# yoyololicon/pytorch-NMF

Measured on AMD Instinct MI355X. Metric: MU GFLOP/s (algorithmic 8*N*C*R per iteration), dense NMF 4096x65536 rank-128 beta=1; MU iterations/s alongside, higher is better.
Workload: dtype f16; 1 GPU; NMF 4096x65536 rank=128 beta=1 (BASELINE configs[1]); preset=cfg1, rows=4096, cols_per_gpu=65536, rank=128, precision=f16, parallelism=single GPU, nsplit_h=16, nsplit_w=1, block_rows_h=256, block_rows_w=256, launch=eager launches

## Files before the change

include/nmfmu.h:

```cpp
#ifndef NMFMU_H_
#define NMFMU_H_

#include <stddef.h>
#include <stdint.h>

#ifdef __cplusplus
extern "C" {
#endif

#define NMFMU_ABI_VERSION 9

#define NMFMU_OK 0
#define NMFMU_ERR_UNSUPPORTED (-2)
#define NMFMU_ERR_ARG (-3)
#define NMFMU_ERR_ALLOC (-4)

#define NMFMU_PREC_BF16 0
#define NMFMU_PREC_BF16X3 1
#define NMFMU_PREC_F16 2
#define NMFMU_PREC_F16X 3
#define NMFMU_PREC_F16R 4

#define NMFMU_BETA_KL 0
#define NMFMU_BETA_EUC 1
#define NMFMU_BETA_IS 2
#define NMFMU_BETA_GEN 3

#define NMFMU_STAGE_REG 0
#define NMFMU_STAGE_DMA 1
#define NMFMU_STAGE_DMA_NOP2 3
#define NMFMU_STAGE_DMA_SPLIT 2

typedef struct nmfmu_factor {
  float* f;
  void* p1_hi;
  void* p1_lo;
  void* p2_hi;
  void* p2_lo;
  float* colsum;
  float* colsum_part;
  int32_t rows;
  int32_t rows_pad;
} nmfmu_factor;

typedef struct nmfmu_step {
// ... 15 lines not shown
  void* stamps;
} nmfmu_step;

int nmfmu_abi_version(void);
int nmfmu_abi_check(int compiled_against);
int nmfmu_pad_rows(int rows);
int nmfmu_pad_rank(int rank);
int nmfmu_beta_kind(float beta);
int nmfmu_supported(int r_pad, int precision);
int nmfmu_block_rows(int r_pad, int precision, float beta);
int nmfmu_choose_nsplit(int owner_rows_pad, int panel_rows_pad, int block_rows, int num_cu);
#define NMFMU_KERNEL_FUSED 0
#define NMFMU_KERNEL_PP 1
#define NMFMU_KERNEL_SP 2
int nmfmu_kernel_family(int r_pad, int precision, float beta);
int nmfmu_choose_nsplit_for(int owner_rows_pad, int panel_rows_pad, int r_pad, int precision, float beta, int block_rows, int num_cu);
int nmfmu_step_block_rows(int owner_rows_pad, int panel_rows_pad, int r_pad, int precision, float beta, int num_cu);
size_t nmfmu_xp_bytes(int owner_rows_pad, int panel_rows_pad, int precision);
size_t nmfmu_image_bytes(int rows_pad, int r_pad);
size_t nmfmu_slab_bytes(int owner_rows_pad, int r_pad, int nsplit);
size_t nmfmu_colsum_part_bytes(int rows_pad, int r_pad);

int nmfmu_pack_x(const float* v, int64_t ld, int rows, int cols, int transpose, int precision, int block_rows, void* xp,
                 int owner_rows_pad, int panel_rows_pad, uint32_t* flags, void* stream);

int nmfmu_pack_factor(const nmfmu_factor* fac, int rank, int r_pad, int precision, void* stream);

int nmfmu_pack_factor_scaled(const nmfmu_factor* fac, int rank, int r_pad, int precision, const float* scale,
                             void* stream);

// ... 244 lines not shown
```

pytorch-nmf_amd/csrc/nmfmu_capi.hip:

```cpp
#include <hip/hip_runtime.h>
#include <stdint.h>

#include <algorithm>
#include <cstdlib>
#include <new>
#include <vector>

#include "../../include/nmfmu.h"
#include "nmfmu_aux.h"
#include "nmfmu_fused.h"
#include "nmfmu_pp.h"
#include "nmfmu_sp.h"
#include "nmfmu_sp2.h"

#ifndef NMFMU_SP
#define NMFMU_SP 1
#endif
#ifndef NMFMU_SP2
#define NMFMU_SP2 1
#endif
#ifndef NMFMU_FUSE_APPLY_TWO_ACC
#define NMFMU_FUSE_APPLY_TWO_ACC 1
#endif

// ... 9 lines not shown

#ifdef NMFMU_DEBUG_HOOKS
static int env_int(const char* name, int dflt) {
  const char* v = std::getenv(name);
  return v && *v ? std::atoi(v) : dflt;
}
static void* g_pp_debug = nullptr;
#endif
#ifndef NMFMU_PP_F16R
#define NMFMU_PP_F16R 1
#endif
static bool pp_eligible(int r_pad, int precision, float beta) {
  return nmfmu_beta_kind(beta) == NMFMU_BETA_KL && r_pad <= 128 &&
         (precision == NMFMU_PREC_F16 || precision == NMFMU_PREC_BF16 || (NMFMU_PP_F16R && precision == NMFMU_PREC_F16R));
}
static bool sp_eligible(int r_pad, int precision, float beta) {
  return NMFMU_SP && nmfmu_beta_kind(beta) == NMFMU_BETA_KL && r_pad == 256 && precision == NMFMU_PREC_F16;
}
static bool sp2_eligible(int r_pad, int precision, float beta) {
  const int k = nmfmu_beta_kind(beta);
  return NMFMU_SP2 && (k == NMFMU_BETA_IS || k == NMFMU_BETA_GEN) && r_pad == 128 && precision == NMFMU_PREC_F16;
}
static int kernel_beta_kind(float beta) {
  if (beta == 0.5f) return kSqrt;
  if (beta == 1.5f) return kSqrt3;
  return nmfmu_beta_kind(beta);
}

struct GramRef {
  const float* gram;
  const void* hi;
  const void* lo;
  const float* scale;
};

int fused_dispatch(const nmfmu_step* st, int mode, float* loss_part, int M, int K, hipStream_t s,
                   const float* fuse_kl_den = nullptr, bool fuse_apply = false, const GramRef* gm = nullptr) {
  if (!st || !st->owner.p1_hi || !st->panel.p1_hi) return NMFMU_ERR_ARG;
  if (!st->xp && (mode == kModeMU || mode == kModeXB)) return NMFMU_ERR_ARG;
  if (st->owner.rows_pad % kRowPad || st->panel.rows_pad % kRowPad) return NMFMU_ERR_ARG;
  if (st->block_rows != 128 && st->block_rows != 256) return NMFMU_ERR_ARG;
  if (st->stage != NMFMU_STAGE_DMA && st->stage != NMFMU_STAGE_DMA_SPLIT && st->stage != NMFMU_STAGE_DMA_NOP2)
    return NMFMU_ERR_UNSUPPORTED;
  if (st->stage == NMFMU_STAGE_DMA_SPLIT && mode == kModeMU && !(st->precision == NMFMU_PREC_BF16X3)) {
    if (nmfmu_beta_kind(st->beta) != NMFMU_BETA_KL || st->block_rows != 128) return NMFMU_ERR_UNSUPPORTED;
    mode = kModeMU2;
  }
  if (st->r_pad != pad_rank(st->rank) || st->nsplit < 1) return NMFMU_ERR_ARG;
  const bool x3 = st->precision == NMFMU_PREC_BF16X3;
  if (x3 && (!st->owner.p1_lo || !st->panel.p1_lo)) return NMFMU_ERR_ARG;
  const int kind = nmfmu_beta_kind(st->beta);
  if (st->precision == NMFMU_PREC_F16R && kind == NMFMU_BETA_EUC) return NMFMU_ERR_UNSUPPORTED;
  FusedArgs a{};
  a.xp = st->xp;
  a.p1_hi = static_cast<const uint16_t*>(st->panel.p1_hi);
  a.p1_lo = static_cast<const uint16_t*>(st->panel.p1_lo);
  a.p2_hi = static_cast<const uint16_t*>(st->panel.p2_hi);
// ... 39 lines not shown
  } else if (mode == kModeMU || mode == kModeDen) {
    if (!a.slab_num || !a.p2_hi || (x3 && !a.p2_lo)) return NMFMU_ERR_ARG;
    if (mode == kModeMU && kind != kKL && !a.slab_den) return NMFMU_ERR_ARG;
    if (mode == kModeDen && (kind != kGen || st->block_rows != 128)) return NMFMU_ERR_UNSUPPORTED;
  } else if (!loss_part) {
    return NMFMU_ERR_ARG;
  }
  const int grid = (st->owner.rows_pad / st->block_rows) * st->nsplit;
  if (st->block_rows == 256) {
    if (!st->xp || mode == kModeDen || !pp_eligible(st->r_pad, st->precision, st->beta)) return NMFMU_ERR_UNSUPPORTED;
    a.tiles_per_split = (a.tiles_per_split + 1) & ~1;
    a.debug = mode == kModeMU ? st->stamps : nullptr;
#ifdef NMFMU_DEBUG_HOOKS
    if (mode == kModeMU && g_pp_debug) a.debug = g_pp_debug;
#endif
    return launch_pp(st->r_pad, is_f16(st->precision) ? kOpF16 : kOpBf16, mode, a, grid, s, st->precision == NMFMU_PREC_F16R,
                      mode == kModeMU && loss_part != nullptr);
  }
  if (mode == kModeMU && sp_eligible(st->r_pad, st->precision, st->beta)) {
    a.tiles_per_split = (a.tiles_per_split + 3) & ~3;
    a.debug = st->stamps;
#ifdef NMFMU_DEBUG_HOOKS
    if (g_pp_debug) a.debug = g_pp_debug;
#endif
    if (st->stage == NMFMU_STAGE_DMA_NOP2) a.o2_hi = nullptr;
    return launch_sp(st->r_pad, kOpF16, a, grid, s);
  }
  if (mode == kModeMU && sp2_eligible(st->r_pad, st->precision, st->beta)) {
    a.tiles_per_split = (a.tiles_per_split + 3) & ~3;
    return launch_sp2(st->r_pad, kernel_beta_kind(st->beta), a, grid, s);
  }
  const int kk = kernel_beta_kind(st->beta);
// ... 52 lines not shown
  static const int forced = env_int("NMFMU_FORCE_NSPLIT", 0);
  if (forced > 0) return std::min(forced, std::max(1, ktiles));
#endif
  const int target = (block_rows == 128 ? 2 : 1) * std::max(num_cu, 1);
  int ns = (target + mblocks - 1) / mblocks;
  if (ns > 8) ns = (ns + 7) / 8 * 8;
  ns = std::min(ns, std::max(1, ktiles / 4));
  return std::max(ns, 1);
}

int nmfmu_kernel_family(int r_pad, int precision, float beta) {
  if (pp_eligible(r_pad, precision, beta)) return NMFMU_KERNEL_PP;
  if (sp_eligible(r_pad, precision, beta) || sp2_eligible(r_pad, precision, beta)) return NMFMU_KERNEL_SP;
  return NMFMU_KERNEL_FUSED;
}

int nmfmu_choose_nsplit_for(int owner_rows_pad, int panel_rows_pad, int r_pad, int precision, float beta, int block_rows, int num_cu) {
  if (owner_rows_pad <= 0 || panel_rows_pad <= 0 || (block_rows != 128 && block_rows != 256)) return NMFMU_ERR_ARG;
  if (block_rows == 128 && (sp_eligible(r_pad, precision, beta) || sp2_eligible(r_pad, precision, beta))) {
    const int mblocks = owner_rows_pad / 128, ktiles = panel_rows_pad / kBK;
    int ns = (std::max(num_cu, 1) + mblocks - 1) / mblocks;
    ns = std::min(ns, std::max(1, ktiles / 8));
    return std::max(ns, 1);
  }
  return nmfmu_choose_nsplit(owner_rows_pad, panel_rows_pad, block_rows, num_cu);
}

int nmfmu_step_block_rows(int owner_rows_pad, int panel_rows_pad, int r_pad, int precision, float beta, int num_cu) {
  if (pp_eligible(r_pad, precision, beta)) return 256;
  if (owner_rows_pad <= 0 || panel_rows_pad <= 0) return NMFMU_ERR_ARG;
// ... 117 lines not shown
  a.nslab = num ? nslab : st->nsplit;
  a.kl_den = kl ? kl_den : nullptr;
  if (!a.num || a.nslab < 1) return NMFMU_ERR_ARG;
  a.den_nslab = den_nslab;
  a.skip_colsum = skip_colsum;
  if (kl ? !a.kl_den : !a.den) return NMFMU_ERR_ARG;
  a.p1_hi = st->owner.p1_hi, a.p1_lo = st->owner.p1_lo, a.p2_hi = st->owner.p2_hi, a.p2_lo = st->owner.p2_lo;
  a.colsum_part = st->owner.colsum_part, a.colsum = st->owner.colsum;
  a.rows = st->owner.rows, a.rank = st->rank, a.rows_pad = st->owner.rows_pad;
  a.l1 = st->l1, a.l2 = st->l2, a.gamma = st->gamma;
  a.trainer = trainer, a.ortho = ortho, a.grad = grad;
  a.f16 = is_f16(st->precision);
  a.status = st->status;
  if (!a.p1_hi || !a.p2_hi || !a.colsum || !a.colsum_part) return NMFMU_ERR_ARG;
  if (st->stage == NMFMU_STAGE_DMA_NOP2 && sp_eligible(st->r_pad, st->precision, st->beta)) a.p2_hi = a.p2_lo = nullptr;
  return launch_apply(st->r_pad, a, st->precision == NMFMU_PREC_BF16X3, false, S(stream));
}

int nmfmu_mu_apply(const nmfmu_step* st, const float* num, const float* den, int nslab, const float* kl_den,
                   void* stream) {
  return apply_common(st, num, den, nslab, kl_den, 0, 0.f, nullptr, stream);
}

int nmfmu_trainer_apply(const nmfmu_step* st, const float* num, const float* den, int nslab, const float* kl_den,
                        float ortho, float* grad, void* stream) {
  if (!(ortho >= 0.f)) return NMFMU_ERR_ARG;
  return apply_common(st, num, den, nslab, kl_den, 1, ortho, grad, stream);
}

int nmfmu_xb_supported(int r_pad, int precision, float beta) {
// ... 233 lines not shown
```

pytorch-nmf_amd/csrc/nmfmu_inst_pp.hip:

```cpp
#include "nmfmu_pp.h"

namespace nmfmu {

bool pp_available(int r_pad, int opt, int mode) {
  return (r_pad == 32 || r_pad == 64 || r_pad == 128) && (opt == kOpBf16 || opt == kOpF16) &&
         (mode == kModeMU || mode == kModeLoss);
}

template <int R_PAD>
static int launch_pp_r(int opt, int mode, const FusedArgs& a, int grid, hipStream_t s, bool xr, bool lacc) {
  if (lacc) {
    if (opt != kOpF16 || mode != kModeMU || !a.loss_part) return -2;
    return xr ? launch_pp_one<R_PAD, kOpF16, kModeMU, true, true>(a, grid, s) : launch_pp_one<R_PAD, kOpF16, kModeMU, false, true>(a, grid, s);
  }
  if (xr) {
    if (opt == kOpF16 && mode == kModeMU) return launch_pp_one<R_PAD, kOpF16, kModeMU, true>(a, grid, s);
    if (opt == kOpF16 && mode == kModeLoss) return launch_pp_one<R_PAD, kOpF16, kModeLoss, true>(a, grid, s);
    return -2;
  }
  if (opt == kOpBf16 && mode == kModeMU) return launch_pp_one<R_PAD, kOpBf16, kModeMU>(a, grid, s);
  if (opt == kOpF16 && mode == kModeMU) return launch_pp_one<R_PAD, kOpF16, kModeMU>(a, grid, s);
  if (opt == kOpBf16 && mode == kModeLoss) return launch_pp_one<R_PAD, kOpBf16, kModeLoss>(a, grid, s);
  if (opt == kOpF16 && mode == kModeLoss) return launch_pp_one<R_PAD, kOpF16, kModeLoss>(a, grid, s);
  return -2;
}

int launch_pp(int r_pad, int opt, int mode, const FusedArgs& a, int grid, hipStream_t s, bool xr, bool lacc) {
  switch (r_pad) {
    case 32: return launch_pp_r<32>(opt, mode, a, grid, s, xr, lacc);
    case 64: return launch_pp_r<64>(opt, mode, a, grid, s, xr, lacc);
    case 128: return launch_pp_r<128>(opt, mode, a, grid, s, xr, lacc);
  }
  return -2;
}

}
```

pytorch-nmf_amd/csrc/nmfmu_pp.h:

```cpp
#pragma once
#include "nmfmu_fused.h"

#ifndef NMFMU_PP_DUP
#define NMFMU_PP_DUP 0
#endif
#ifndef NMFMU_PP_XM
#define NMFMU_PP_XM -1
#endif

namespace nmfmu {

template <int R_PAD, int OPT, int MODE, bool XR_ = false, bool LACC_ = false>
struct PPCfg {
  static constexpr int BM = 256, WAVES = 8, THREADS = 512;
  static constexpr int KS = R_PAD / 16;
  static constexpr int RT = R_PAD / 32;
  static constexpr int ROWB = 2 * R_PAD;
  static constexpr int IMG = kBK * ROWB;
  static constexpr bool LOSS = MODE == kModeLoss;
  static constexpr int LEAD = 2;
  static constexpr int NSLOT = 3;
  static constexpr bool XR = XR_;
  static constexpr int NX = XR ? 6 : 4;
  static constexpr int XTILE = BM * kBK * (XR ? 3 : 2);
  static_assert(!XR || OPT == kOpF16, "the 3-byte target comes with fp16 operands");
  static constexpr bool LACC = LACC_;
  static_assert(!LACC || (OPT == kOpF16 && MODE == kModeMU), "riding loss: fp16 operands, MU half-step");
  static constexpr bool XM = (NMFMU_PP_DUP & (4 | 32)) ? false : (NMFMU_PP_XM < 0 ? XR : NMFMU_PP_XM != 0);
  static constexpr int P1_BASE = 0, P2_BASE = NSLOT * IMG;
  static constexpr int LDS_MAIN = 2 * NSLOT * IMG;
  static constexpr int LDS_EPI = LOSS ? 64 : WAVES * 32 * R_PAD * 4;
  static constexpr int LDS_BYTES = LDS_MAIN > LDS_EPI ? LDS_MAIN : LDS_EPI;
  static constexpr int NPIECE = IMG / 1024;
  static constexpr int ND = (NPIECE + 3) / 4;
  static constexpr int NSTEP1 = 2 * KS, NSTEP2 = LOSS ? 0 : 4 * RT;
  static constexpr int PF = 4;
  static constexpr bool SCALED = OPT == kOpBf16;
  static_assert(NSTEP1 >= PF, "ring deeper than G1");
};

template <int R_PAD, int OPT, int MODE, bool XR = false, bool LACC = false>
__global__ void __launch_bounds__(512, 2) pp_kernel(const FusedArgs a) {
  using C = PPCfg<R_PAD, OPT, MODE, XR, LACC>;
  constexpr int NX = C::NX;
  constexpr int KS = C::KS, RT = C::RT, ROWB = C::ROWB, IMG = C::IMG, PF = C::PF;
  constexpr int NSTEP1 = C::NSTEP1, NSTEP2 = C::NSTEP2;
  extern __shared__ __attribute__((aligned(16))) char smem[];

  const int tid = threadIdx.x;
  const int lane = tid & 63;
  const int wave = __builtin_amdgcn_readfirstlane(tid >> 6);
  const int half = wave >> 2;
  const int j = lane & 31;
  const int hl = lane >> 5;
  const int mb = blockIdx.x / a.nsplit;
  const int ks = blockIdx.x - mb * a.nsplit;
  const int t0 = ks * a.tiles_per_split;
  const int t1 = min(t0 + a.tiles_per_split, a.ktiles);
// ... 93 lines not shown
#pragma unroll
      for (int i = 0; i < C::ND; ++i) {
        const unsigned pc = (4u * i) % (unsigned)C::NPIECE;
        if constexpr (C::NPIECE >= 4)
          dma1k(src_tile + pc * 1024u, pvoff, lds_base + lds_off + pc * 1024u + (unsigned)(wave & 3) * 1024u);
        else
          dma1k(src_tile, ((unsigned)(wave & 3) % (unsigned)C::NPIECE) * 1024u + lane16,
                lds_base + lds_off + ((unsigned)(wave & 3) % (unsigned)C::NPIECE) * 1024u);
      }
    };
    unsigned p1_issue_off = (unsigned)(C::LEAD % C::NSLOT) * IMG;
    unsigned p2_issue_off = (unsigned)((C::LEAD - 1) % C::NSLOT) * IMG;
    auto next_off = [&](unsigned off) { return off == (unsigned)(C::NSLOT - 1) * IMG ? 0u : off + IMG; };
    auto issue_panel = [&](int t) {
      dma_img(p1src + (size_t)clampt(t + C::LEAD) * IMG, C::P1_BASE + p1_issue_off);
      if constexpr (!C::LOSS) dma_img(p2src + (size_t)clampt(t + C::LEAD - 1) * IMG, C::P2_BASE + p2_issue_off);
    };
#ifdef NMFMU_PP_X_DEFAULT_POLICY
#define NMFMU_PP_XPOL ""
#else
#define NMFMU_PP_XPOL " nt"
#endif
    u32x4 xA[NX], xB[NX];
#if NMFMU_PP_DUP & (4 | 32)
    u32x4 xdupA[4], xdupB[4];
#if NMFMU_PP_DUP & 32
    const long long xmirror = (long long)((int)(gridDim.x / a.nsplit) - 1 - 2 * mb) * (long long)a.ktiles * (long long)C::XTILE;
#else
    const long long xmirror = 0;
#endif
#endif
// ... 70 lines not shown
    uint32_t gn[2][8];
    f32x16 S[2];
    u32x4 ring[PF];
#ifdef NMFMU_PP_ABLATE_STALE_OPERANDS
    u32x4 abl_sink = {0u, 0u, 0u, 0u};
#endif

    constexpr int BACK = (C::NSLOT - 1) * IMG;
    int sa[2] = {a_base[0] + C::P1_BASE, a_base[1] + C::P1_BASE};
    int sb[2][2];
#pragma unroll
    for (int tt = 0; tt < 2; ++tt)
#pragma unroll
      for (int m2 = 0; m2 < 2; ++m2) sb[tt][m2] = b_base[tt][m2] + C::P2_BASE + BACK;
    int rd1 = 0, rd2 = BACK;
    auto advance_slots = [&]() {
      const int d1 = rd1 == BACK ? -BACK : IMG;
      const int d2 = rd2 == BACK ? -BACK : IMG;
      rd1 += d1, rd2 += d2;
      sa[0] += d1, sa[1] += d1;
      if constexpr (!C::LOSS) {
#pragma unroll
        for (int tt = 0; tt < 2; ++tt)
#pragma unroll
          for (int m2 = 0; m2 < 2; ++m2) sb[tt][m2] += d2;
      }
    };
    auto rd = [&](u32x4& dst, int addr, auto offc) {
#if NMFMU_PP_DUP & 1
      asm volatile("ds_read_b128 %0, %1 offset:%2\n\tds_read_b128 %0, %1 offset:%2" : "=v"(dst) : "v"(addr), "n"(decltype(offc)::value));
#else
      asm volatile("ds_read_b128 %0, %1 offset:%2" : "=v"(dst) : "v"(addr), "n"(decltype(offc)::value));
#endif
    };
    auto opnd = [&](u32x4& dst, auto ec, auto g1c) {
// ... 74 lines not shown
          mma(acc[rt], nh, op);
        }
        if constexpr (e + PF < NS) opnd(ring[e % PF], std::integral_constant<int, e + PF>{}, g1c);
        if constexpr (decltype(fillc)::value) {
          static_for<NX>([&](auto ic) {
            if constexpr ((decltype(ic)::value * NS) / NX == e) fill(ic);
          });
        }
      });
      if constexpr (g1 && N2 == 0) asm volatile("s_nop 15\n\ts_nop 7" ::: "memory");
    };
    auto elementwise_segment = [&](int t, auto nextc, u32x4(&x)[NX], auto tailc) {
      constexpr bool next_has_g1 = decltype(nextc)::value;
      constexpr bool tail = decltype(tailc)::value;
      advance_slots();
      if constexpr (next_has_g1) prefetch(std::true_type{});
      else if constexpr (!C::LOSS) prefetch(std::false_type{});
      if constexpr (!tail) {
        if (!half) issue_panel(t);
      } else if constexpr (next_has_g1 && !C::LOSS) {
        if (!half) dma_img(p2src + (size_t)(t + 1) * IMG, C::P2_BASE + p2_issue_off);
      }
#pragma unroll
      for (int tt = 0; tt < 2; ++tt) {
        if constexpr (C::LOSS) {
#pragma unroll
          for (int d = 0; d < 8; ++d) {
            const uint32_t w = x[2 * tt + (d >> 2)][d & 3];
            float x0, x1;
            if constexpr (C::XR) {
              const uint32_t uw = x[4 + tt][d >> 1], j0 = 2 * (d & 1);
              x0 = __builtin_bit_cast(float, __builtin_amdgcn_perm(w, uw, 0x0504000cu | (j0 << 8)));
              x1 = __builtin_bit_cast(float, __builtin_amdgcn_perm(w, uw, 0x0706000cu | ((j0 + 1) << 8)));
            } else {
              x0 = unpack_lo<OPT>(w), x1 = unpack_hi<OPT>(w);
            }
            const int k0 = (t0 + t) * kBK + 32 * hl + 16 * tt + 2 * d;
            const bool rowok = m0 < a.M;
            constexpr float un = SCALED ? 1.1920928955078125e-07f : 1.f;
// ... 112 lines not shown
          }
        } else {
#pragma unroll
          for (int d = 0; d < 8; ++d) {
            const uint32_t w = x[2 * tt + (d >> 2)][d & 3];
            const float n0 = bf16_lo(w) * __builtin_amdgcn_rcpf(S[tt][2 * d]);
            const float n1 = bf16_hi(w) * __builtin_amdgcn_rcpf(S[tt][2 * d + 1]);
            gn[tt][d] = pack_bf16(n0, n1);
          }
        }
      }
      p1_issue_off = next_off(p1_issue_off);
      p2_issue_off = next_off(p2_issue_off);
      __builtin_amdgcn_sched_barrier(0);
      if constexpr (!tail && !C::XM) load_x(t + 2, x);
    };

    if (!half) {
#pragma unroll
      for (int i = 0; i < C::LEAD; ++i) dma_img(p1src + (size_t)clampt(i) * IMG, C::P1_BASE + i * IMG);
      if constexpr (!C::LOSS) {
#pragma unroll
        for (int i = 0; i < C::LEAD - 1; ++i) dma_img(p2src + (size_t)clampt(i) * IMG, C::P2_BASE + i * IMG);
      }
    }
    load_x(0, xA);
    load_x(1, xB);
    load_owner();
    asm volatile("s_waitcnt vmcnt(0)"
                 : "+v"(xA[0]), "+v"(xA[1]), "+v"(xA[2]), "+v"(xA[3]), "+v"(xB[0]), "+v"(xB[1]), "+v"(xB[2]), "+v"(xB[3])::"memory");
    tie_x(xA);
    tie_x(xB);
#if NMFMU_PP_DUP & (4 | 32)
    asm volatile("" : "+v"(xdupA[0]), "+v"(xdupA[1]), "+v"(xdupA[2]), "+v"(xdupA[3]), "+v"(xdupB[0]), "+v"(xdupB[1]), "+v"(xdupB[2]), "+v"(xdupB[3]));
#endif
    scale_owner();
    barrier();
    prefetch(std::true_type{});
    if (half) barrier();
    matrix_segment(std::true_type{}, std::false_type{}, std::false_type{}, no_fill);
    stamp(0);
    auto tile_full = [&](int t, u32x4(&xc)[NX], u32x4(&xn)[NX], auto tailc) {
      constexpr bool tail = decltype(tailc)::value;
      barrier();
      elementwise_segment(t, std::true_type{}, xc, tailc);
      barrier();
      if constexpr (!tail && C::XM) {
        const char* src = xsrc + (size_t)clampt(t + 2) * (size_t)C::XTILE;
        const char* src4 = src + 4096;
        asm volatile("" : "+s"(src), "+s"(src4));
        matrix_segment(std::true_type{}, std::true_type{}, std::true_type{}, [&](auto ic) { load_x1(ic, xc, src, src4); });
      } else {
// ... 145 lines not shown
#pragma unroll
            for (int k = 0; k < 4; ++k)
              if (r0 + 4 * h + k < a.rank) frow[4 * h + k] = fv[4 * h + k];
          }
        }
        *reinterpret_cast<float4*>(trow) = *reinterpret_cast<const float4*>(fv);
        *reinterpret_cast<float4*>(trow + 4) = *reinterpret_cast<const float4*>(fv + 4);
        u32x4 hi;
#pragma unroll
        for (int qq = 0; qq < 4; ++qq) hi[qq] = pack_op<OPT>(fv[2 * qq], fv[2 * qq + 1]);
        *reinterpret_cast<u32x4*>(reinterpret_cast<char*>(a.o1_hi) + p1_offset(row, r0, R_PAD)) = hi;
      }
      if constexpr (OPT == kOpF16) {
        if (a.status && __any(clamped) && lane_e == 0) atomicOr(a.status, 1u);
      }
      __syncthreads();
#pragma unroll
      for (int ii = 0; ii < R_PAD / 64 + (R_PAD < 64 ? 1 : 0); ++ii) {
        const int r = ii * 64 + lane_e;
        if (r < R_PAD) {
#pragma unroll
          for (int g = 0; g < 4; ++g) {
            const float* src = tile + (g * 8) * LDT + r;
            u32x4 hi;
#pragma unroll
            for (int qq = 0; qq < 4; ++qq) hi[qq] = pack_op<OPT>(src[(2 * qq) * LDT], src[(2 * qq + 1) * LDT]);
            *reinterpret_cast<u32x4*>(reinterpret_cast<char*>(a.o2_hi) + p2_offset(mrow0 + g * 8, r, R_PAD)) = hi;
          }
        }
      }
      __syncthreads();
      float* red = reinterpret_cast<float*>(smem);
#pragma unroll
      for (int k = 0; k < 8; ++k) {
        float tot = csum8[k];
        if constexpr (SP <= 32) tot += __shfl_xor(tot, 32, 64);
        if constexpr (SP <= 16) tot += __shfl_xor(tot, 16, 64);
        if constexpr (SP <= 8) tot += __shfl_xor(tot, 8, 64);
        if constexpr (SP <= 4) tot += __shfl_xor(tot, 4, 64);
        if (lane_e < SP) red[wave * R_PAD + slot_e * 8 + k] = tot;
      }
      __syncthreads();
// ... 8 lines not shown
        constexpr int rt = decltype(rtc)::value;
#pragma unroll
        for (int e = 0; e < 16; ++e) {
          const int row = (e & 3) + 8 * (e >> 2) + 4 * hl_e;
          a.slab_num[slab + (size_t)row * R_PAD + rt * 32 + j_e] = acc[rt][e];
        }
      });
    }
  }
  if constexpr (MODE == kModeMU) {
    if (a.debug) asm volatile("s_waitcnt vmcnt(0)" ::: "memory");
    stamp(3);
  }
}

template <int R_PAD, int OPT, int MODE, bool XR = false, bool LACC = false>
int launch_pp_one(const FusedArgs& a, int grid, hipStream_t s) {
  using C = PPCfg<R_PAD, OPT, MODE, XR, LACC>;
  return launch_with_dynamic_lds<pp_kernel<R_PAD, OPT, MODE, XR, LACC>, C::THREADS, C::LDS_BYTES>(dim3(grid), s, a);
}

int launch_pp(int r_pad, int opt, int mode, const FusedArgs& a, int grid, hipStream_t s, bool xr = false, bool lacc = false);
bool pp_available(int r_pad, int opt, int mode);

}
```

pytorch-nmf_amd/torchnmf_amd/_capi.py:

```python
from __future__ import annotations

import ctypes as C
import os
from typing import Optional

LIB_NAME = 'libnmfmu.so'
LIB_PATH = os.environ.get('NMFMU_LIB') or os.path.join(os.path.dirname(os.path.abspath(__file__)), LIB_NAME)

OK = 0
ERR_UNSUPPORTED = -2
ERR_ARG = -3
ERR_ALLOC = -4
PREC_BF16, PREC_BF16X3, PREC_F16, PREC_F16X, PREC_F16R = 0, 1, 2, 3, 4
STAGE_REG, STAGE_DMA, STAGE_DMA_SPLIT = 0, 1, 2
STAGE_DMA_NOP2 = 3
BETA_KL, BETA_EUC, BETA_IS, BETA_GEN = 0, 1, 2, 3
KERNEL_FUSED, KERNEL_PP, KERNEL_SP = 0, 1, 2

PRECISIONS = {'bf16': PREC_BF16, 'bf16x3': PREC_BF16X3, 'f16': PREC_F16, 'f16x': PREC_F16X, 'f16r': PREC_F16R}


class NmfmuError(RuntimeError):
    pass


class Factor(C.Structure):
    _fields_ = [('f', C.c_void_p), ('p1_hi', C.c_void_p), ('p1_lo', C.c_void_p), ('p2_hi', C.c_void_p),
                ('p2_lo', C.c_void_p), ('colsum', C.c_void_p), ('colsum_part', C.c_void_p), ('rows', C.c_int32),
                ('rows_pad', C.c_int32)]

# ... 20 lines not shown
ABI_VERSION = 9
EPI_RATIO, EPI_F32, EPI_LOSS, EPI_FOLD = 0, 1, 2, 3
OPS_PLANES, OPS_B_HU, OPS_B_HUT, OPS_A_HU, OPS_A_WIN = 0, 1, 2, 3, 4

SIGNATURES = {
    'nmfmu_abi_version': (C.c_int, []),
    'nmfmu_abi_check': (C.c_int, [C.c_int]),
    'nmfmu_pad_rows': (C.c_int, [C.c_int]),
    'nmfmu_pad_rank': (C.c_int, [C.c_int]),
    'nmfmu_beta_kind': (C.c_int, [C.c_float]),
    'nmfmu_supported': (C.c_int, [C.c_int, C.c_int]),
    'nmfmu_block_rows': (C.c_int, [C.c_int, C.c_int, C.c_float]),
    'nmfmu_step_block_rows': (C.c_int, [C.c_int, C.c_int, C.c_int, C.c_int, C.c_float, C.c_int]),
    'nmfmu_choose_nsplit': (C.c_int, [C.c_int, C.c_int, C.c_int, C.c_int]),
    'nmfmu_kernel_family': (C.c_int, [C.c_int, C.c_int, C.c_float]),
    'nmfmu_choose_nsplit_for': (C.c_int, [C.c_int, C.c_int, C.c_int, C.c_int, C.c_float, C.c_int, C.c_int]),
    'nmfmu_xp_bytes': (C.c_size_t, [C.c_int, C.c_int, C.c_int]),
    'nmfmu_image_bytes': (C.c_size_t, [C.c_int, C.c_int]),
    'nmfmu_slab_bytes': (C.c_size_t, [C.c_int, C.c_int, C.c_int]),
    'nmfmu_colsum_part_bytes': (C.c_size_t, [C.c_int, C.c_int]),
    'nmfmu_pack_x': (C.c_int, [C.c_void_p, C.c_int64, C.c_int, C.c_int, C.c_int, C.c_int, C.c_int, C.c_void_p,
                               C.c_int, C.c_int, C.c_void_p, C.c_void_p]),
    'nmfmu_pack_factor': (C.c_int, [C.POINTER(Factor), C.c_int, C.c_int, C.c_int, C.c_void_p]),
    'nmfmu_mu_partial': (C.c_int, [C.POINTER(Step), C.c_void_p]),
    'nmfmu_den_partial': (C.c_int, [C.POINTER(Step), C.c_void_p]),
    'nmfmu_mu_step': (C.c_int, [C.POINTER(Step), C.c_void_p, C.c_int, C.c_void_p]),
    'nmfmu_xb_supported': (C.c_int, [C.c_int, C.c_int, C.c_float]),
    'nmfmu_gram_ws_bytes': (C.c_size_t, [C.c_int]),
    'nmfmu_gram_panel': (C.c_int, [C.POINTER(Factor), C.c_int, C.c_int, C.c_void_p, C.c_void_p, C.c_void_p, C.c_void_p,
                                   C.c_void_p, C.c_void_p]),
# ... 180 lines not shown
```

pytorch-nmf_amd/torchnmf_amd/engine.py:

```python
from __future__ import annotations

import ctypes as C
import os
from typing import Optional

import torch

from . import _capi


def _ptr(t: Optional[torch.Tensor]) -> Optional[int]:
    return None if t is None else t.data_ptr()


class HipBackend:

    name = 'hip'

    def __init__(self):
        self.lib = _capi.load()
        if not torch.cuda.is_available():
            raise _capi.NmfmuError('torchnmf_amd needs a ROCm device (MI355X); none is visible and there is no '
                                   'CPU fallback')

# ... 17 lines not shown
        if br not in (128, 256):
            _capi.check(br if br < 0 else _capi.ERR_ARG, 'nmfmu_step_block_rows')
        return br

    def choose_nsplit(self, m_pad: int, k_pad: int, block_rows: int, device, r_pad=None, precision=None, beta=None) -> int:
        ncu = torch.cuda.get_device_properties(device).multi_processor_count
        forced = os.environ.get('TORCHNMF_AMD_NSPLIT')
        if forced:
            return max(1, min(int(forced), k_pad // 64 // 4))
        if r_pad is not None:
            return self.lib.nmfmu_choose_nsplit_for(m_pad, k_pad, r_pad, precision, beta, block_rows, ncu)
        return self.lib.nmfmu_choose_nsplit(m_pad, k_pad, block_rows, ncu)

    def kernel_family(self, r_pad: int, precision: int, beta: float) -> int:
        return self.lib.nmfmu_kernel_family(r_pad, precision, beta)

    @staticmethod
    def stream() -> int:
        return torch.cuda.current_stream().cuda_stream

    def alloc(self, nbytes: int, device) -> torch.Tensor:
        return torch.empty(max(int(nbytes), 16), dtype=torch.uint8, device=device)

    def pack_x(self, V, transpose, precision, block_rows, m_pad, k_pad, flags, out=None):
        xp = out if out is not None else self.alloc(self.lib.nmfmu_xp_bytes(m_pad, k_pad, precision), V.device)
        _capi.check(self.lib.nmfmu_pack_x(V.data_ptr(), V.stride(0), V.shape[0], V.shape[1], int(transpose), precision,
                                          block_rows, xp.data_ptr(), m_pad, k_pad, _ptr(flags), self.stream()),
                    'nmfmu_pack_x')
        return xp

# ... 382 lines not shown
                        f"(fp16 operands -- 'f16', or 'f16x' with an fp32 target -- need both dimensions >= {self.F16_MIN_DIM} "
                        f"and data within fp16's range; split bf16 stops at rank 128); pass precision='bf16' (factors "
                        f"~1e-3), 'f16' or 'f16x' explicitly")
                precision = 'bf16x3'
        if precision not in _capi.PRECISIONS:
            raise ValueError(f"precision must be one of {sorted(_capi.PRECISIONS)} or 'auto', got {precision!r}")
        self.precision_name = precision
        self.precision = _capi.PRECISIONS[precision]
        if not self.be.supported(self.r_pad, self.precision):
            raise NotImplementedError(f'precision {precision!r} is not available for rank {R} (padded {self.r_pad})')
        if stage is None:
            nop2 = (hasattr(self.be, 'kernel_family') and hasattr(_capi, 'STAGE_DMA_NOP2') and float(beta) == 1.0
                    and self.r_pad == 256 and self.be.kernel_family(self.r_pad, self.precision, float(beta)) == _capi.KERNEL_SP
                    and os.environ.get('TORCHNMF_AMD_NO_P2', '1') != '0')
            stage = _capi.STAGE_DMA_NOP2 if nop2 else _capi.STAGE_DMA
        self.gram_path = (allow_gram and self.beta == 2.0 and group is None and block_rows in (None, 128)
                          and hasattr(self.be, 'xb_supported') and self.be.xb_supported(self.r_pad, self.precision, self.beta)
                          and os.environ.get('TORCHNMF_AMD_BETA2_GRAM', '1') != '0')
        gamma = mu_gamma(self.beta)
        dev = V.device

        self.fW = FactorBuf(W, self.r_pad, self.precision, self.be)
        self.fH = FactorBuf(H, self.r_pad, self.precision, self.be)
        self.flags = torch.tensor([0, 0x7f800000], dtype=torch.int32, device=dev)
        self.status = torch.zeros(1, dtype=torch.int32, device=dev)
        n_pad, c_pad = self.fH.rows_pad, self.fW.rows_pad
        def tile_rows(m_pad, k_pad):
            if block_rows is not None:
                return block_rows
            if hasattr(self.be, 'step_block_rows'):
# ... 246 lines not shown
```

Before: 892,900 GFLOP/s.

## Build the transposed panel image in LDS instead of storing and DMA-ing P2

Adds an LDS-transpose stage for the rank-128 PP kernel. The second (transposed) panel image is now derived in shared memory from the P1 image using ds_read_b64_tr_b16 reads and ds_write_b64 writes, which are overlapped with the MFMA loop. This removes the P2 DMA loads, the kernel's o2 transposed-output writes, and the P2 pack in apply. In exchange it adds LDS traffic and lgkm waits inside the main loop, and the Python side selects this stage by default for eligible configs.

```diff
diff --git a/include/nmfmu.h b/include/nmfmu.h
--- a/include/nmfmu.h
+++ b/include/nmfmu.h
@@ -29,6 +29,7 @@
 #define NMFMU_STAGE_REG 0
 #define NMFMU_STAGE_DMA 1
 #define NMFMU_STAGE_DMA_NOP2 3
+#define NMFMU_STAGE_DMA_LDSTR 4
 #define NMFMU_STAGE_DMA_SPLIT 2
 
 typedef struct nmfmu_factor {
@@ -74,6 +75,7 @@
 #define NMFMU_KERNEL_PP 1
 #define NMFMU_KERNEL_SP 2
 int nmfmu_kernel_family(int r_pad, int precision, float beta);
+int nmfmu_pp_lds_transpose_supported(int r_pad, int precision, float beta);
 int nmfmu_choose_nsplit_for(int owner_rows_pad, int panel_rows_pad, int r_pad, int precision, float beta, int block_rows, int num_cu);
 int nmfmu_step_block_rows(int owner_rows_pad, int panel_rows_pad, int r_pad, int precision, float beta, int num_cu);
 size_t nmfmu_xp_bytes(int owner_rows_pad, int panel_rows_pad, int precision);
diff --git a/pytorch-nmf_amd/csrc/nmfmu_capi.hip b/pytorch-nmf_amd/csrc/nmfmu_capi.hip
--- a/pytorch-nmf_amd/csrc/nmfmu_capi.hip
+++ b/pytorch-nmf_amd/csrc/nmfmu_capi.hip
@@ -47,6 +47,9 @@
   return nmfmu_beta_kind(beta) == NMFMU_BETA_KL && r_pad <= 128 &&
          (precision == NMFMU_PREC_F16 || precision == NMFMU_PREC_BF16 || (NMFMU_PP_F16R && precision == NMFMU_PREC_F16R));
 }
+static bool pp_ldstr_eligible(int r_pad, int precision, float beta) {
+  return pp_eligible(r_pad, precision, beta) && pp_trl_available(r_pad, is_f16(precision) ? kOpF16 : kOpBf16, kModeMU);
+}
 static bool sp_eligible(int r_pad, int precision, float beta) {
   return NMFMU_SP && nmfmu_beta_kind(beta) == NMFMU_BETA_KL && r_pad == 256 && precision == NMFMU_PREC_F16;
 }
@@ -73,7 +76,11 @@
   if (!st->xp && (mode == kModeMU || mode == kModeXB)) return NMFMU_ERR_ARG;
   if (st->owner.rows_pad % kRowPad || st->panel.rows_pad % kRowPad) return NMFMU_ERR_ARG;
   if (st->block_rows != 128 && st->block_rows != 256) return NMFMU_ERR_ARG;
-  if (st->stage != NMFMU_STAGE_DMA && st->stage != NMFMU_STAGE_DMA_SPLIT && st->stage != NMFMU_STAGE_DMA_NOP2)
+  if (st->stage != NMFMU_STAGE_DMA && st->stage != NMFMU_STAGE_DMA_SPLIT && st->stage != NMFMU_STAGE_DMA_NOP2 &&
+      st->stage != NMFMU_STAGE_DMA_LDSTR)
+    return NMFMU_ERR_UNSUPPORTED;
+  const bool ldstr = st->stage == NMFMU_STAGE_DMA_LDSTR && mode != kModeLoss;
+  if (ldstr && (mode != kModeMU || st->block_rows != 256 || !pp_ldstr_eligible(st->r_pad, st->precision, st->beta)))
     return NMFMU_ERR_UNSUPPORTED;
   if (st->stage == NMFMU_STAGE_DMA_SPLIT && mode == kModeMU && !(st->precision == NMFMU_PREC_BF16X3)) {
     if (nmfmu_beta_kind(st->beta) != NMFMU_BETA_KL || st->block_rows != 128) return NMFMU_ERR_UNSUPPORTED;
@@ -143,8 +150,9 @@
 #ifdef NMFMU_DEBUG_HOOKS
     if (mode == kModeMU && g_pp_debug) a.debug = g_pp_debug;
 #endif
+    if (ldstr) a.o2_hi = nullptr;
     return launch_pp(st->r_pad, is_f16(st->precision) ? kOpF16 : kOpBf16, mode, a, grid, s, st->precision == NMFMU_PREC_F16R,
-                      mode == kModeMU && loss_part != nullptr);
+                      mode == kModeMU && loss_part != nullptr, ldstr);
   }
   if (mode == kModeMU && sp_eligible(st->r_pad, st->precision, st->beta)) {
     a.tiles_per_split = (a.tiles_per_split + 3) & ~3;
@@ -227,6 +235,8 @@
   if (sp_eligible(r_pad, precision, beta) || sp2_eligible(r_pad, precision, beta)) return NMFMU_KERNEL_SP;
   return NMFMU_KERNEL_FUSED;
 }
+
+int nmfmu_pp_lds_transpose_supported(int r_pad, int precision, float beta) { return pp_ldstr_eligible(r_pad, precision, beta) ? 1 : 0; }
 
 int nmfmu_choose_nsplit_for(int owner_rows_pad, int panel_rows_pad, int r_pad, int precision, float beta, int block_rows, int num_cu) {
   if (owner_rows_pad <= 0 || panel_rows_pad <= 0 || (block_rows != 128 && block_rows != 256)) return NMFMU_ERR_ARG;
@@ -374,6 +384,10 @@
   a.status = st->status;
   if (!a.p1_hi || !a.p2_hi || !a.colsum || !a.colsum_part) return NMFMU_ERR_ARG;
   if (st->stage == NMFMU_STAGE_DMA_NOP2 && sp_eligible(st->r_pad, st->precision, st->beta)) a.p2_hi = a.p2_lo = nullptr;
+  if (st->stage == NMFMU_STAGE_DMA_LDSTR) {
+    if (st->block_rows != 256 || !pp_ldstr_eligible(st->r_pad, st->precision, st->beta)) return NMFMU_ERR_UNSUPPORTED;
+    a.p2_hi = a.p2_lo = nullptr;
+  }
   return launch_apply(st->r_pad, a, st->precision == NMFMU_PREC_BF16X3, false, S(stream));
 }
 
diff --git a/pytorch-nmf_amd/csrc/nmfmu_inst_pp.hip b/pytorch-nmf_amd/csrc/nmfmu_inst_pp.hip
--- a/pytorch-nmf_amd/csrc/nmfmu_inst_pp.hip
+++ b/pytorch-nmf_amd/csrc/nmfmu_inst_pp.hip
@@ -5,6 +5,21 @@
 bool pp_available(int r_pad, int opt, int mode) {
   return (r_pad == 32 || r_pad == 64 || r_pad == 128) && (opt == kOpBf16 || opt == kOpF16) &&
          (mode == kModeMU || mode == kModeLoss);
+}
+
+bool pp_trl_available(int r_pad, int opt, int mode) {
+  return r_pad == 128 && (opt == kOpBf16 || opt == kOpF16) && mode == kModeMU;
+}
+
+static int launch_pp_trl(int opt, const FusedArgs& a, int grid, hipStream_t s, bool xr, bool lacc) {
+  if (lacc) {
+    if (opt != kOpF16 || !a.loss_part) return -2;
+    return xr ? launch_pp_one<128, kOpF16, kModeMU, true, true, true>(a, grid, s) : launch_pp_one<128, kOpF16, kModeMU, false, true, true>(a, grid, s);
+  }
+  if (xr) return opt == kOpF16 ? launch_pp_one<128, kOpF16, kModeMU, true, false, true>(a, grid, s) : -2;
+  if (opt == kOpBf16) return launch_pp_one<128, kOpBf16, kModeMU, false, false, true>(a, grid, s);
+  if (opt == kOpF16) return launch_pp_one<128, kOpF16, kModeMU, false, false, true>(a, grid, s);
+  return -2;
 }
 
 template <int R_PAD>
@@ -25,7 +40,8 @@
   return -2;
 }
 
-int launch_pp(int r_pad, int opt, int mode, const FusedArgs& a, int grid, hipStream_t s, bool xr, bool lacc) {
+int launch_pp(int r_pad, int opt, int mode, const FusedArgs& a, int grid, hipStream_t s, bool xr, bool lacc, bool trl) {
+  if (trl) return pp_trl_available(r_pad, opt, mode) ? launch_pp_trl(opt, a, grid, s, xr, lacc) : -2;
   switch (r_pad) {
     case 32: return launch_pp_r<32>(opt, mode, a, grid, s, xr, lacc);
     case 64: return launch_pp_r<64>(opt, mode, a, grid, s, xr, lacc);
diff --git a/pytorch-nmf_amd/csrc/nmfmu_pp.h b/pytorch-nmf_amd/csrc/nmfmu_pp.h
--- a/pytorch-nmf_amd/csrc/nmfmu_pp.h
+++ b/pytorch-nmf_amd/csrc/nmfmu_pp.h
@@ -10,7 +10,7 @@
 
 namespace nmfmu {
 
-template <int R_PAD, int OPT, int MODE, bool XR_ = false, bool LACC_ = false>
+template <int R_PAD, int OPT, int MODE, bool XR_ = false, bool LACC_ = false, bool TRL_ = false>
 struct PPCfg {
   static constexpr int BM = 256, WAVES = 8, THREADS = 512;
   static constexpr int KS = R_PAD / 16;
@@ -26,6 +26,8 @@
   static_assert(!XR || OPT == kOpF16, "the 3-byte target comes with fp16 operands");
   static constexpr bool LACC = LACC_;
   static_assert(!LACC || (OPT == kOpF16 && MODE == kModeMU), "riding loss: fp16 operands, MU half-step");
+  static constexpr bool TRL = TRL_;
+  static_assert(!TRL || (MODE == kModeMU && R_PAD == 128), "transpose in LDS: MU half-step at padded rank 128");
   static constexpr bool XM = (NMFMU_PP_DUP & (4 | 32)) ? false : (NMFMU_PP_XM < 0 ? XR : NMFMU_PP_XM != 0);
   static constexpr int P1_BASE = 0, P2_BASE = NSLOT * IMG;
   static constexpr int LDS_MAIN = 2 * NSLOT * IMG;
@@ -39,9 +41,9 @@
   static_assert(NSTEP1 >= PF, "ring deeper than G1");
 };
 
-template <int R_PAD, int OPT, int MODE, bool XR = false, bool LACC = false>
+template <int R_PAD, int OPT, int MODE, bool XR = false, bool LACC = false, bool TRL = false>
 __global__ void __launch_bounds__(512, 2) pp_kernel(const FusedArgs a) {
-  using C = PPCfg<R_PAD, OPT, MODE, XR, LACC>;
+  using C = PPCfg<R_PAD, OPT, MODE, XR, LACC, TRL>;
   constexpr int NX = C::NX;
   constexpr int KS = C::KS, RT = C::RT, ROWB = C::ROWB, IMG = C::IMG, PF = C::PF;
   constexpr int NSTEP1 = C::NSTEP1, NSTEP2 = C::NSTEP2;
@@ -165,7 +167,7 @@
     auto next_off = [&](unsigned off) { return off == (unsigned)(C::NSLOT - 1) * IMG ? 0u : off + IMG; };
     auto issue_panel = [&](int t) {
       dma_img(p1src + (size_t)clampt(t + C::LEAD) * IMG, C::P1_BASE + p1_issue_off);
-      if constexpr (!C::LOSS) dma_img(p2src + (size_t)clampt(t + C::LEAD - 1) * IMG, C::P2_BASE + p2_issue_off);
+      if constexpr (!C::LOSS && !C::TRL) dma_img(p2src + (size_t)clampt(t + C::LEAD - 1) * IMG, C::P2_BASE + p2_issue_off);
     };
 #ifdef NMFMU_PP_X_DEFAULT_POLICY
 #define NMFMU_PP_XPOL ""
@@ -266,11 +268,41 @@
 #pragma unroll
       for (int m2 = 0; m2 < 2; ++m2) sb[tt][m2] = b_base[tt][m2] + C::P2_BASE + BACK;
     int rd1 = 0, rd2 = BACK;
+    int tr_src = 0, tr_dst = 0;
+    if constexpr (C::TRL) {
+      const int rt = wave & 3, tt = wave >> 2, grp = lane >> 4, s16 = lane & 15, i4 = s16 >> 2;
+      const int cslot = 2 * (grp & 1) + ((s16 & 3) >> 1);
+      tr_src = C::P1_BASE + (32 * (grp >> 1) + 16 * tt + i4) * ROWB + (((((rt ^ i4) << 2) | cslot) << 4) + 8 * (s16 & 1));
+      tr_dst = C::P2_BASE + (32 * rt + j) * 128 + (((4 * hl + 2 * tt) ^ ((j >> 1) & 7)) << 4);
+    }
+    using u32x2 = __attribute__((ext_vector_type(2))) uint32_t;
+    u32x2 trv[4];
+    auto tr_rd = [&](u32x2& dst, int addr, auto offc) {
+      asm volatile("ds_read_b64_tr_b16 %0, %1 offset:%2" : "=v"(dst) : "v"(addr), "n"(decltype(offc)::value));
+    };
+    auto tr_wr = [&](const u32x2& v, int addr, auto offc) {
+      asm volatile("ds_write_b64 %0, %1 offset:%2" ::"v"(addr), "v"(v), "n"(decltype(offc)::value) : "memory");
+    };
+    auto transpose_read = [&]() {
+      tr_rd(trv[0], tr_src, std::integral_constant<int, 0>{});
+      tr_rd(trv[1], tr_src ^ 16, std::integral_constant<int, 4 * ROWB>{});
+      tr_rd(trv[2], tr_src ^ 32, std::integral_constant<int, 8 * ROWB>{});
+      tr_rd(trv[3], tr_src ^ 48, std::integral_constant<int, 12 * ROWB>{});
+    };
+    auto transpose_write = [&]() {
+      asm volatile("s_waitcnt lgkmcnt(0)" : "+v"(trv[0]), "+v"(trv[1]), "+v"(trv[2]), "+v"(trv[3])::"memory");
+      tr_wr(trv[0], tr_dst, std::integral_constant<int, 0>{});
+      tr_wr(trv[1], tr_dst, std::integral_constant<int, 8>{});
+      tr_wr(trv[2], tr_dst ^ 16, std::integral_constant<int, 0>{});
+      tr_wr(trv[3], tr_dst ^ 16, std::integral_constant<int, 8>{});
+    };
+    auto transpose_done = [&]() { asm volatile("s_waitcnt lgkmcnt(0)" ::: "memory"); };
     auto advance_slots = [&]() {
       const int d1 = rd1 == BACK ? -BACK : IMG;
       const int d2 = rd2 == BACK ? -BACK : IMG;
       rd1 += d1, rd2 += d2;
       sa[0] += d1, sa[1] += d1;
+      if constexpr (C::TRL) tr_src += d1, tr_dst += d1;
       if constexpr (!C::LOSS) {
 #pragma unroll
         for (int tt = 0; tt < 2; ++tt)
@@ -375,15 +407,23 @@
       constexpr bool next_has_g1 = decltype(nextc)::value;
       constexpr bool tail = decltype(tailc)::value;
       advance_slots();
+      constexpr bool trl = C::TRL && next_has_g1;
+      if constexpr (trl) transpose_read();
       if constexpr (next_has_g1) prefetch(std::true_type{});
       else if constexpr (!C::LOSS) prefetch(std::false_type{});
       if constexpr (!tail) {
         if (!half) issue_panel(t);
-      } else if constexpr (next_has_g1 && !C::LOSS) {
+      } else if constexpr (next_has_g1 && !C::LOSS && !C::TRL) {
         if (!half) dma_img(p2src + (size_t)(t + 1) * IMG, C::P2_BASE + p2_issue_off);
       }
 #pragma unroll
       for (int tt = 0; tt < 2; ++tt) {
+        if constexpr (trl) {
+          if (tt == 1) {
+            __builtin_amdgcn_sched_barrier(0);
+            transpose_write();
+          }
+        }
         if constexpr (C::LOSS) {
 #pragma unroll
           for (int d = 0; d < 8; ++d) {
@@ -526,12 +566,13 @@
       p2_issue_off = next_off(p2_issue_off);
       __builtin_amdgcn_sched_barrier(0);
       if constexpr (!tail && !C::XM) load_x(t + 2, x);
+      if constexpr (trl) transpose_done();
     };
 
     if (!half) {
 #pragma unroll
       for (int i = 0; i < C::LEAD; ++i) dma_img(p1src + (size_t)clampt(i) * IMG, C::P1_BASE + i * IMG);
-      if constexpr (!C::LOSS) {
+      if constexpr (!C::LOSS && !C::TRL) {
 #pragma unroll
         for (int i = 0; i < C::LEAD - 1; ++i) dma_img(p2src + (size_t)clampt(i) * IMG, C::P2_BASE + i * IMG);
       }
@@ -548,6 +589,11 @@
 #endif
     scale_owner();
     barrier();
+    if constexpr (C::TRL) {
+      transpose_read();
+      transpose_write();
+      transpose_done();
+    }
     prefetch(std::true_type{});
     if (half) barrier();
     matrix_segment(std::true_type{}, std::false_type{}, std::false_type{}, no_fill);
@@ -723,18 +769,20 @@
       if constexpr (OPT == kOpF16) {
         if (a.status && __any(clamped) && lane_e == 0) atomicOr(a.status, 1u);
       }
-      __syncthreads();
-#pragma unroll
-      for (int ii = 0; ii < R_PAD / 64 + (R_PAD < 64 ? 1 : 0); ++ii) {
-        const int r = ii * 64 + lane_e;
-        if (r < R_PAD) {
-#pragma unroll
-          for (int g = 0; g < 4; ++g) {
-            const float* src = tile + (g * 8) * LDT + r;
-            u32x4 hi;
-#pragma unroll
-            for (int qq = 0; qq < 4; ++qq) hi[qq] = pack_op<OPT>(src[(2 * qq) * LDT], src[(2 * qq + 1) * LDT]);
-            *reinterpret_cast<u32x4*>(reinterpret_cast<char*>(a.o2_hi) + p2_offset(mrow0 + g * 8, r, R_PAD)) = hi;
+      if (a.o2_hi) {
+        __syncthreads();
+#pragma unroll
+        for (int ii = 0; ii < R_PAD / 64 + (R_PAD < 64 ? 1 : 0); ++ii) {
+          const int r = ii * 64 + lane_e;
+          if (r < R_PAD) {
+#pragma unroll
+            for (int g = 0; g < 4; ++g) {
+              const float* src = tile + (g * 8) * LDT + r;
+              u32x4 hi;
+#pragma unroll
+              for (int qq = 0; qq < 4; ++qq) hi[qq] = pack_op<OPT>(src[(2 * qq) * LDT], src[(2 * qq + 1) * LDT]);
+              *reinterpret_cast<u32x4*>(reinterpret_cast<char*>(a.o2_hi) + p2_offset(mrow0 + g * 8, r, R_PAD)) = hi;
+            }
           }
         }
       }
@@ -773,13 +821,15 @@
   }
 }
 
-template <int R_PAD, int OPT, int MODE, bool XR = false, bool LACC = false>
+template <int R_PAD, int OPT, int MODE, bool XR = false, bool LACC = false, bool TRL = false>
 int launch_pp_one(const FusedArgs& a, int grid, hipStream_t s) {
-  using C = PPCfg<R_PAD, OPT, MODE, XR, LACC>;
-  return launch_with_dynamic_lds<pp_kernel<R_PAD, OPT, MODE, XR, LACC>, C::THREADS, C::LDS_BYTES>(dim3(grid), s, a);
+  using C = PPCfg<R_PAD, OPT, MODE, XR, LACC, TRL>;
+  return launch_with_dynamic_lds<pp_kernel<R_PAD, OPT, MODE, XR, LACC, TRL>, C::THREADS, C::LDS_BYTES>(dim3(grid), s, a);
 }
 
-int launch_pp(int r_pad, int opt, int mode, const FusedArgs& a, int grid, hipStream_t s, bool xr = false, bool lacc = false);
+int launch_pp(int r_pad, int opt, int mode, const FusedArgs& a, int grid, hipStream_t s, bool xr = false, bool lacc = false,
+              bool trl = false);
 bool pp_available(int r_pad, int opt, int mode);
+bool pp_trl_available(int r_pad, int opt, int mode);
 
 }
diff --git a/pytorch-nmf_amd/torchnmf_amd/_capi.py b/pytorch-nmf_amd/torchnmf_amd/_capi.py
--- a/pytorch-nmf_amd/torchnmf_amd/_capi.py
+++ b/pytorch-nmf_amd/torchnmf_amd/_capi.py
@@ -14,6 +14,7 @@
 PREC_BF16, PREC_BF16X3, PREC_F16, PREC_F16X, PREC_F16R = 0, 1, 2, 3, 4
 STAGE_REG, STAGE_DMA, STAGE_DMA_SPLIT = 0, 1, 2
 STAGE_DMA_NOP2 = 3
+STAGE_DMA_LDSTR = 4
 BETA_KL, BETA_EUC, BETA_IS, BETA_GEN = 0, 1, 2, 3
 KERNEL_FUSED, KERNEL_PP, KERNEL_SP = 0, 1, 2
 
@@ -64,6 +65,7 @@
     'nmfmu_step_block_rows': (C.c_int, [C.c_int, C.c_int, C.c_int, C.c_int, C.c_float, C.c_int]),
     'nmfmu_choose_nsplit': (C.c_int, [C.c_int, C.c_int, C.c_int, C.c_int]),
     'nmfmu_kernel_family': (C.c_int, [C.c_int, C.c_int, C.c_float]),
+    'nmfmu_pp_lds_transpose_supported': (C.c_int, [C.c_int, C.c_int, C.c_float]),
     'nmfmu_choose_nsplit_for': (C.c_int, [C.c_int, C.c_int, C.c_int, C.c_int, C.c_float, C.c_int, C.c_int]),
     'nmfmu_xp_bytes': (C.c_size_t, [C.c_int, C.c_int, C.c_int]),
     'nmfmu_image_bytes': (C.c_size_t, [C.c_int, C.c_int]),
diff --git a/pytorch-nmf_amd/torchnmf_amd/engine.py b/pytorch-nmf_amd/torchnmf_amd/engine.py
--- a/pytorch-nmf_amd/torchnmf_amd/engine.py
+++ b/pytorch-nmf_amd/torchnmf_amd/engine.py
@@ -55,6 +55,9 @@
 
     def kernel_family(self, r_pad: int, precision: int, beta: float) -> int:
         return self.lib.nmfmu_kernel_family(r_pad, precision, beta)
+
+    def pp_lds_transpose_supported(self, r_pad: int, precision: int, beta: float) -> bool:
+        return bool(self.lib.nmfmu_pp_lds_transpose_supported(r_pad, precision, beta))
 
     @staticmethod
     def stream() -> int:
@@ -467,6 +470,10 @@
                     and self.r_pad == 256 and self.be.kernel_family(self.r_pad, self.precision, float(beta)) == _capi.KERNEL_SP
                     and os.environ.get('TORCHNMF_AMD_NO_P2', '1') != '0')
             stage = _capi.STAGE_DMA_NOP2 if nop2 else _capi.STAGE_DMA
+            if (group is None and update_W and block_rows in (None, 256) and hasattr(self.be, 'pp_lds_transpose_supported')
+                    and self.be.pp_lds_transpose_supported(self.r_pad, self.precision, float(beta))
+                    and self.be.block_rows(self.r_pad, self.precision, float(beta)) == 256):
+                stage = _capi.STAGE_DMA_LDSTR
         self.gram_path = (allow_gram and self.beta == 2.0 and group is None and block_rows in (None, 128)
                           and hasattr(self.be, 'xb_supported') and self.be.xb_supported(self.r_pad, self.precision, self.beta)
                           and os.environ.get('TORCHNMF_AMD_BETA2_GRAM', '1') != '0')
```

New measurement: 911,800 GFLOP/s, median of 6. +2.1%, better.
